# penumbra-zone/decaf377

Measured on AMD Instinct MI355X. Metric: decaf377 var-base scalar-mults/sec + encodes/sec at 1/2/4/8 MI355X, higher is better.
Workload: dtype u32

## Files before the change

decaf377_amd/csrc/curve.hpp:

```cpp
#pragma once
#include "fq29.hpp"
#include "fqs29.hpp"

namespace d377 {

#include "constants.inc"

constexpr int GT_STRIDE = 12;
constexpr int S_HASH_BITS = 12;
struct SqrtTables {
  const uint32_t* gtab;
  const uint8_t* s_lookup;
  uint32_t* inv_fail;
};

#include "s_hash.inc"

D377_HD uint32_t s_hash_raw(const fe& x) {
  return ((x.l[0] ^ (x.l[1] << 3)) * D377_S_HASH_K) >> (32 - S_HASH_BITS);
}
D377_HD uint32_t s_hash(const fe& x) {
  D377_B(bound_require(x.vq < 1.0535, "s_lookup key must be below q + 2^248"));
  return s_hash_raw(x);
}

D377_HD fe gt_load(const SqrtTables& T, int table, uint32_t idx) {
  const uint32_t* p = T.gtab + ((size_t)table * 256 + idx) * GT_STRIDE;
  fe r;
#if defined(__HIP_DEVICE_COMPILE__)
  const uint4* p4 = reinterpret_cast<const uint4*>(p);
  uint4 a = p4[0], b = p4[1], c = p4[2];
  r.l[0] = a.x; r.l[1] = a.y; r.l[2] = a.z; r.l[3] = a.w;
  r.l[4] = b.x; r.l[5] = b.y; r.l[6] = b.z; r.l[7] = b.w;
  r.l[8] = c.x;
#else
  for (int i = 0; i < NL; ++i) r.l[i] = p[i];
#endif
  fe_assume_carried(r, 1.1);
  return r;
}

D377_HD fe fe_sqr_n(fe x, int n) {
#pragma unroll 1
  for (int i = 0; i + 1 < n; i += 2) x = fe_sqr(fe_sqr(x));
  if (n & 1) x = fe_sqr(x);
  return x;
}

D377_HD fe fe_pow_2_47_m1(const fe& x) {
  fe e2 = fe_mul(fe_sqr(x), x);
  fe e4 = fe_mul(fe_sqr_n(e2, 2), e2);
  fe e5 = fe_mul(fe_sqr(e4), x);
  fe e10 = fe_mul(fe_sqr_n(e5, 5), e5);
  fe e11 = fe_mul(fe_sqr(e10), x);
  fe e22 = fe_mul(fe_sqr_n(e11, 11), e11);
  fe e23 = fe_mul(fe_sqr(e22), x);
  fe e46 = fe_mul(fe_sqr_n(e23, 23), e23);
  return fe_mul(fe_sqr(e46), x);
}

#ifndef D377_POW_W
#define D377_POW_W 4
#endif
#if D377_POW_W == 3
#define D377_POW_CHAIN POW_M12_CHAIN_W3
// ... 4 lines not shown
#define D377_POW_LEN D377_POW_M12_W4_LEN
#define D377_POW_TRAIL D377_POW_M12_W4_TRAILING_SQ
#endif
constexpr int POW_TAB = 1 << (D377_POW_W - 1);

struct RegPowTab {
  fe t[8];
  D377_HD void put(int j, const fe& v) { t[j] = v; }
  D377_HD fe get(int j) const {
    fe f;
    switch (j) {
      case 0: f = t[0]; break;
      case 1: f = t[1]; break;
      case 2: f = t[2]; break;
      case 3: f = t[3]; break;
      case 4: f = t[4]; break;
      case 5: f = t[5]; break;
      case 6: f = t[6]; break;
      default: f = t[7]; break;
    }
    return f;
  }
};

template <class PT>
D377_HD fe fe_pow_m12(const fe& x, PT& pt) {
  fe x2 = fe_sqr(x);
  fe cur = x;
  pt.put(0, cur);
#pragma unroll 1
  for (int j = 1; j < POW_TAB; ++j) {
    cur = fe_mul(cur, x2);
    pt.put(j, cur);
  }
  fe acc = pt.get((int)(D377_POW_CHAIN[0] & 15u) >> 1);
#pragma unroll 1
  for (int i = 1; i < D377_POW_LEN; ++i) {
    const uint32_t e = D377_POW_CHAIN[i];
    acc = fe_sqr_n(acc, (int)(e >> 4));
    acc = fe_mul(acc, pt.get((int)(e & 15u) >> 1));
  }
  return fe_sqr_n(acc, D377_POW_TRAIL);
}

D377_HD bool fe_strict_is_zero(const fe& a) {
  D377_B(bound_require(a.vq < 2.0, "fe_strict_is_zero needs a value below 2q"));
  uint32_t o = 0, d = 0;
#pragma unroll
  for (int i = 0; i < NL; ++i) { o |= a.l[i]; d |= a.l[i] ^ QL[i]; }
  return o == 0 || d == 0;
}

D377_HD bool fe_sqrt_tail(const SqrtTables& T, const fe& v, const fe& uv, bool den_zero, bool num_zero, fe* res, bool min_curve_root);

struct GivenPowers {
  fe v, uv;
  D377_HD void put(int, const fe&) {}
  D377_HD fe get(int) const { return fe_zero(); }
};
template <class PT> struct pt_has_powers { static constexpr bool value = false; };
template <> struct pt_has_powers<GivenPowers> { static constexpr bool value = true; };

template <bool NUM_IS_ONE, class PT>
D377_HD bool fe_sqrt_ratio_zeta(const SqrtTables& T, PT& pt, const fe& num, const fe& den, fe* res,
                                bool min_curve_root = false, const fe* inv_den = nullptr, bool use_inv = true) {
  const bool den_zero = fe_strict_is_zero(den);
  bool num_zero = false;
  if (!NUM_IS_ONE) num_zero = fe_strict_is_zero(num);

  fe v, uv;
  if constexpr (pt_has_powers<PT>::value) {
    v = pt.v;
    uv = pt.uv;
  } else if (inv_den != nullptr && use_inv) {
    const fe z = NUM_IS_ONE ? *inv_den : fe_mul(num, *inv_den);
    v = fe_pow_m12(z, pt);
    uv = fe_mul(v, z);
  } else {
    fe s = fe_pow_2_47_m1(den);
    fe t_ = fe_mul(fe_sqr(s), den);
    fe w = NUM_IS_ONE ? fe_mul(fe_pow_m12(t_, pt), s)
                      : fe_mul(fe_pow_m12(fe_mul(num, t_), pt), s);
    v = fe_mul(w, den);
    uv = NUM_IS_ONE ? w : fe_mul(w, num);
  }
  return fe_sqrt_tail(T, v, uv, den_zero, num_zero, res, min_curve_root);
}
D377_HD bool fe_sqrt_tail(const SqrtTables& T, const fe& v, const fe& uv, bool den_zero, bool num_zero, fe* res, bool min_curve_root) {
  fe x5 = fe_mul(uv, v);
  fe x4 = fe_sqr_n(x5, 8);
  fe x3 = fe_sqr_n(x4, 8);
  fe x2 = fe_sqr_n(x3, 8);
  fe x1 = fe_sqr_n(x2, 8);
  fe x0 = fe_sqr_strict(fe_sqr_strict(fe_sqr_n(x1, 5)));

  const uint64_t q0p = T.s_lookup[s_hash(x0)];
  uint64_t t = q0p;
  fe a1 = fe_mul_strict(x1, gt_load(T, 4, (uint32_t)(t & 0xFF)));
  t += (uint64_t)T.s_lookup[s_hash(a1)] << 7;
  fe a2 = fe_mul_strict(fe_mul(x2, gt_load(T, 3, (uint32_t)(t & 0xFF))),
                        gt_load(T, 4, (uint32_t)((t >> 8) & 0xFF)));
  t += (uint64_t)T.s_lookup[s_hash(a2)] << 15;
  fe a3 = fe_mul_strict(fe_mul(fe_mul(x3, gt_load(T, 2, (uint32_t)(t & 0xFF))),
                               gt_load(T, 3, (uint32_t)((t >> 8) & 0xFF))),
                        gt_load(T, 4, (uint32_t)((t >> 16) & 0xFF)));
  t += (uint64_t)T.s_lookup[s_hash(a3)] << 23;
  fe a4 = fe_mul_strict(fe_mul(fe_mul(fe_mul(x4, gt_load(T, 1, (uint32_t)(t & 0xFF))),
                                      gt_load(T, 2, (uint32_t)((t >> 8) & 0xFF))),
                               gt_load(T, 3, (uint32_t)((t >> 16) & 0xFF))),
                        gt_load(T, 4, (uint32_t)((t >> 24) & 0xFF)));
  t += (uint64_t)T.s_lookup[s_hash(a4)] << 31;
  fe a5 = fe_mul_strict(fe_mul(fe_mul(fe_mul(fe_mul(x5, gt_load(T, 0, (uint32_t)(t & 0xFF))),
                                             gt_load(T, 1, (uint32_t)((t >> 8) & 0xFF))),
                                      gt_load(T, 2, (uint32_t)((t >> 16) & 0xFF))),
                               gt_load(T, 3, (uint32_t)((t >> 24) & 0xFF))),
                        gt_load(T, 4, (uint32_t)((t >> 32) & 0xFF)));
  t += (uint64_t)T.s_lookup[s_hash(a5)] << 39;

  const uint64_t e2 = (D377_TS_U_INV * (t >> 1)) & ((1ull << 46) - 1);
  const bool flip = min_curve_root && (((D377_TS_U * e2) >> 46) & 1ull) != 0;
  t = (t + 1) >> 1;
  const bool nonsq = (q0p & 1) != 0;
  fe r = fe_select(nonsq, fe_mul(uv, fe_const(FE_NONSQUARE)), uv);
  r = fe_mul(r, gt_load(T, 0, (uint32_t)(t & 0xFF)));
  r = fe_mul(r, gt_load(T, 1, (uint32_t)((t >> 8) & 0xFF)));
  r = fe_mul(r, gt_load(T, 2, (uint32_t)((t >> 16) & 0xFF)));
  r = fe_mul(r, gt_load(T, 3, (uint32_t)((t >> 24) & 0xFF)));
  r = fe_mul(r, gt_load(T, 4, (uint32_t)((t >> 32) & 0xFF)));
  r = fe_mul(r, gt_load(T, 5, (uint32_t)((t >> 40) & 0xFF)));

  if (min_curve_root) r = fe_select(flip, fe_neg(r), r);
  bool was_square = !nonsq;
  if (den_zero) { r = fe_zero(); was_square = false; }
  if (num_zero) { r = fe_zero(); was_square = true; }
  *res = r;
  return was_square;
}

D377_HD fe fe_from_words_mod_order(const uint32_t w[8]) {
  return fe_mul(fe_from_words(w), fe_const(FE_R2));
}
D377_HD fe fe_from_words_mod_order_strict(const uint32_t w[8]) {
  return fe_mul_strict(fe_from_words(w), fe_const(FE_R2));
}
D377_HD fe fe_from_wide_words(const uint32_t lo[8], const uint32_t hi[8]) {
  return fe_add(fe_mul(fe_from_words(lo), fe_const(FE_R2)), fe_mul(fe_from_words(hi), fe_const(FE_R2_SHIFT256)));
}
D377_HD void fe_to_limbs28(const fe& x, uint32_t rec16[16]) {
  uint32_t w[8];
  fe_to_words(fe_canon(x), w);
#pragma unroll
  for (int k = 0; k < 10; ++k) {
    const int bit = 28 * k, lo = bit >> 5, sh = bit & 31;
// ... 275 lines not shown
}
template <class SQRT>
D377_HD uint32_t ge_decompress_with(const SqrtTables& T, const uint32_t w[8], ge* out, SQRT sqrt_of) {
  uint32_t bad = (w[7] >> 29) != 0;
  bad |= (uint32_t)words_geq(w, FQ_MODULUS_W_LIT);
  bad |= (w[0] & 1u);
  fe s = fe_mul(fe_from_words(w), fe_const(FE_R2));
  fe ss = fe_sqr(s);
  fe u1 = fe_sub(fe_const(FE_ONE), ss);
  fe u1sq = fe_sqr_strict(u1);
  fe u2 = fe_sub(u1sq, fe_mul(fe_const(FE_4D), ss));
  fe v;
  const bool was_square = sqrt_of(fe_mul_strict(u2, u1sq), &v);
  bad |= (uint32_t)!was_square;
  fe two_s_u1 = fe_mul(fe_dbl(s), u1);
  if (fe_is_negative(fe_mul(two_s_u1, v))) v = fe_neg(v);
  out->x = fe_mul(fe_mul(two_s_u1, fe_sqr(v)), u2);
  out->y = fe_mul(fe_mul(fe_add(fe_const(FE_ONE), ss), v), u1);
  out->z = fe_const(FE_ONE);
  out->t = fe_mul(out->x, out->y);
  D377_INVARIANT(T, *out, bad == 0);
  return bad;
}
template <class PT>
D377_HD uint32_t ge_decompress(const SqrtTables& T, PT& pt, const uint32_t w[8], ge* out, const fe* inv_den = nullptr) {
  return ge_decompress_with(T, w, out, [&](const fe& den, fe* v) {
    return fe_sqrt_ratio_zeta<true>(T, pt, fe_zero(), den, v, false, inv_den);
  });
}
D377_HD uint32_t ge_decompress_from_powers(const SqrtTables& T, const uint32_t w[8], const fe& pv, const fe& puv, ge* out) {
  return ge_decompress_with(T, w, out, [&](const fe& den, fe* v) {
    return fe_sqrt_tail(T, pv, puv, fe_strict_is_zero(den), false, v, false);
  });
}

D377_HD fe ge_compress_den(const ge& p) {
  fe u1 = fe_mul(fe_add(p.x, p.t), fe_sub(p.x, p.t));
  return fe_mul_strict(fe_mul(u1, fe_const(FE_A_MINUS_D)), fe_sqr(p.x));
}
template <class PT>
D377_HD void ge_compress(const SqrtTables& T, PT& pt, const ge& p, uint32_t w[8], bool is_element = true,
                         const fe* inv_den = nullptr) {
  D377_INVARIANT(T, p, is_element);
  const fe a_minus_d = fe_const(FE_A_MINUS_D);
  fe u1 = fe_mul(fe_add(p.x, p.t), fe_sub(p.x, p.t));
  fe v;
  (void)fe_sqrt_ratio_zeta<true>(T, pt, fe_zero(), fe_mul_strict(fe_mul(u1, a_minus_d), fe_sqr(p.x)), &v, false, inv_den);
  fe u2 = fe_abs(fe_mul(v, u1));
  fe u3 = fe_sub(fe_mul(u2, p.z), p.t);
  fe s = fe_mul(fe_mul(fe_mul(a_minus_d, v), u3), p.x);
// ... 218 lines not shown
  return r;
}

template <class F>
D377_HD ge_of<F> ge_double_neg(const ge_of<F>& p, bool with_t) {
  F a = fe_sqr(p.x), b = fe_sqr(p.y);
  F c = fe_sqr2x(p.z);
  F e = fe_mul(p.x, fe_dbl(p.y));
  F h = fe_add(a, b);
  F g = fe_sub(a, b);
  F f = fe_add(g, c);
  ge_of<F> r;
  r.x = fe_mul(e, f); r.y = fe_mul(g, h); r.z = fe_mul(f, g);
  r.t = p.t;
  if (with_t) r.t = fe_mul(e, h);
  return r;
}

D377_HD ge ge_double_latency(const ge& p) { return ge_double_fast(p, true); }

template <class F>
D377_HD gec_of<F> ge_to_cached(const ge_of<F>& p) {
  gec_of<F> c;
  c.ypx = fe_carry(fe_add(p.y, p.x));
  c.ymx = fe_sub(p.y, p.x);
  c.z2 = fe_dbl(p.z);
  c.kt = fe_mul(fe_as<F>(fe_const(FE_K)), p.t);
  return c;
}

template <class F>
D377_HD ge_of<F> ge_add_cached(const ge_of<F>& p, const gec_of<F>& q, bool neg, bool with_t) {
  F a = fe_mul(fe_sub_nc(p.y, p.x), q.ymx);
  F b = fe_mul(fe_add(p.y, p.x), q.ypx);
  F c = fe_mul(p.t, q.kt);
  F d = fe_mul(p.z, q.z2);
  F e = fe_sub(b, a), h = fe_add(b, a);
  F dmc = fe_sub(d, c), dpc = fe_add(d, c);
  F f = fe_select(neg, dpc, dmc), g = fe_select(neg, dmc, dpc);
  ge_of<F> r;
  r.x = fe_mul(e, f); r.y = fe_mul(g, h); r.z = fe_mul(f, g);
  r.t = p.t;
  if (with_t) r.t = fe_mul(e, h);
  return r;
}

struct gea { fe ypx, ymx, kt; };
// ... 10 lines not shown
  r.t = p.t;
  if (with_t) r.t = fe_mul(e, h);
  return r;
}

D377_HD gea gea_from_affine(const fe& x, const fe& y) {
  gea c;
  c.ypx = fe_carry(fe_add(y, x));
  c.ymx = fe_sub(y, x);
  c.kt = fe_mul(fe_mul(fe_const(FE_K), x), y);
  return c;
}
D377_HD ge ge_from_cached_affine(const gea& q, bool neg) {
  const fe one = fe_const(FE_ONE);
  ge r;
  r.x = fe_mul(fe_sub(q.ypx, fe_mul(q.ymx, one)), one);
  r.y = fe_mul(fe_add(q.ypx, q.ymx), one);
  r.z = fe_const(FE_TWO);
  const fe t = fe_mul(q.kt, fe_const(FE_2_OVER_K));
  r.t = fe_select(neg, fe_neg(t), t);
  return r;
}

template <class F = fe, class Tab>
D377_HD ge ge_scalar_mul_w4(const ge& p0, const uint32_t digits[8], Tab& tab, bool want_t = true) {
  const ge_of<F> p = ge_as<F>(p0);
  {
    gec_of<F> id;
    id.ypx = fe_as<F>(fe_const(FE_ONE)); id.ymx = fe_as<F>(fe_const(FE_ONE)); id.z2 = fe_dbl(fe_as<F>(fe_const(FE_ONE)));
    id.kt = fe_as<F>(fe_zero());
    tab.store(0, id);
  }
  const gec_of<F> pc = ge_to_cached(p);
  tab.store(1, pc);
  ge_of<F> acc = ge_double_fast(p, true);
  tab.store(2, ge_to_cached(acc));
#pragma unroll 1
  for (int j = 3; j <= 8; ++j) {
    acc = ge_add_cached(acc, pc, false, true);
    tab.store(j, ge_to_cached(acc));
  }
  int d = fr_digit(digits, 63);
  ge_of<F> r = ge_as<F>(ge_select(d != 0, p0, ge_identity()));
#pragma unroll 1
  for (int i = 62; i >= 0; --i) {
    d = fr_digit(digits, i);
    const bool neg = d < 0;
    const gec_of<F> e = tab.load(neg ? -d : d, neg);
#pragma unroll 1
    for (int j = 0; j < 4; ++j) r = ge_double_neg(r, j == 3);
    r = ge_add_cached(r, e, neg, want_t && i == 0);
  }
  return ge_unsigned(r);
}

// ... 302 lines not shown
```

decaf377_amd/csrc/d377.hip:

```cpp
#include <hip/hip_runtime.h>
#include <stdint.h>
#include <stdio.h>
#include <stdlib.h>
#include <string.h>
#include <chrono>
#include <mutex>
#include <new>
#include <string>
#include <thread>
#include <type_traits>
#include <vector>

#include "../../include/decaf377_amd.h"
#include "curve.hpp"
#include "device_util.hpp"
#include "dcb.hpp"
#include "quad_ops.hpp"
#include "row_ops.hpp"
#include "host_state.hpp"
#include "codec_chunked.hpp"
#include "fixed_comb.hpp"

using namespace d377;

thread_local char d377_g_err[512] = "";

namespace {

template <class F>
struct GlobalTab {
  uint32_t* base;
  size_t nthreads, tid;
  __device__ __forceinline__ void store(int j, const gec_of<F>& c) {
    uint32_t* p = base + ((size_t)j * nthreads + tid) * VB_ENTRY_WORDS;
    slot_store(p, c.ypx); slot_store(p + SLOT, c.ymx); slot_store(p + 2 * SLOT, c.z2); slot_store(p + 3 * SLOT, c.kt);
  }
  __device__ __forceinline__ gec_of<F> load(int j, bool swap) const {
    const uint32_t* p = base + ((size_t)j * nthreads + tid) * VB_ENTRY_WORDS;
    gec_of<F> c;
    c.ypx = slot_load_as<F>(p + (swap ? SLOT : 0));
    c.ymx = slot_load_as<F>(p + (swap ? 0 : SLOT));
    c.z2 = slot_load_as<F>(p + 2 * SLOT);
    c.kt = slot_load_as<F>(p + 3 * SLOT);
    return c;
  }
};
template <int BITS>
struct FixedTab {
  const uint32_t* base;
  __device__ __forceinline__ gea load(int i, int j, bool swap) const {
    return pt_load_affine(base + ((size_t)i * FbShape<BITS>::entries + j) * FBW_ENTRY_WORDS, swap);
  }
};

__device__ fe fe_pow_u32(const fe& x, uint32_t e) {
  int top = 31 - __clz((int)e);
  fe r = x;
#pragma unroll 1
  for (int i = top - 1; i >= 0; --i) {
    r = fe_sqr(r);
    if ((e >> i) & 1u) r = fe_mul(r, x);
  }
  return r;
}

__global__ void __launch_bounds__(BLOCK) k_init_gtab(uint32_t* gtab) {
  const int idx = blockIdx.x * BLOCK + threadIdx.x;
  if (idx >= 6 * 256) return;
  const int t = idx >> 8, nu = idx & 255;
  fe base = fe_sqr_n(fe_const(FE_SQRT_G), 8 * t);
  fe v = nu == 0 ? fe_const(FE_ONE) : fe_pow_u32(base, (uint32_t)nu);
  v = fe_mul_strict(v, fe_const(FE_ONE));
  uint32_t* p = gtab + (size_t)idx * GT_STRIDE;
#pragma unroll
  for (int i = 0; i < NL; ++i) p[i] = v.l[i];
  p[9] = 0; p[10] = 0; p[11] = 0;
}

__global__ void __launch_bounds__(BLOCK) k_init_slookup(uint8_t* s_lookup, uint32_t* keys ,
                                                        int* collisions) {
  const int nu = threadIdx.x;
  fe b39 = fe_sqr_n(fe_const(FE_SQRT_G_INV), 39);
  fe v = nu == 0 ? fe_const(FE_ONE) : fe_pow_u32(b39, (uint32_t)nu);
  fe c = fe_reduce_once(fe_mul_strict(v, fe_const(FE_ONE)));
  keys[2 * nu] = s_hash_raw(c);
  uint32_t h2 = 0xFFFFFFFFu;
  if (c.l[NL - 1] < (1u << 16)) {
    fe cq = fe_add(c, fe_const(Q_LIMBS));
    uint32_t carry = 0;
    fe n;
#pragma unroll
    for (int i = 0; i < NL; ++i) {
      uint32_t t = cq.l[i] + carry;
      if (i < NL - 1) { n.l[i] = t & MASK29; carry = t >> RB; } else n.l[i] = t;
    }
    h2 = s_hash_raw(n);
  }
  keys[2 * nu + 1] = h2;
  for (int i = threadIdx.x; i < (1 << S_HASH_BITS); i += BLOCK) s_lookup[i] = 0;
// ... 204 lines not shown
        io.put(3, j, w);
      }
    },
    [&](DcbIO& io2, int cnt) {
      if (__any(flagged != 0)) {
#pragma unroll 1
        for (int j = 0; j < cnt; ++j) {
          const bool mine = ((flagged >> j) & 1u) != 0;
          if (!__any(mine)) continue;
          Words8 a1, a2;
          io2.get(2, j, a1.w);
          io2.get(3, j, a2.w);
          const Words8 r = hash_exceptional_words(T, pt, a1, a2);
          if (mine) io2.emit(j, r.w);
        }
      }
      flagged = 0;
    });
  D377_DCB_END();
}

__global__ void __launch_bounds__(BLOCK, WAVES_PER_SIMD) k_scalar_mul_var(SqrtTables T, const uint8_t* enc32,
                                                          const uint8_t* scalar32, size_t n, uint8_t* out32,
                                                          uint8_t* status, uint32_t* scratch, DcbScratch dcb) {
  D377_POW_LDS();
  D377_DCB_BEGIN(out32);
  GlobalTab<fes> tab;
  tab.base = scratch;
  tab.nthreads = (size_t)dcb.nslots * BLOCK;
  tab.tid = io.lane;
  dcb_rounds<1, true, false>(n, io, pt,
    [&](size_t i, int j) {
      uint32_t w[8];
      load32(enc32, i, w);
      dcb_put_den(io, 0, j, ge_decompress_den(w));
    },
    [&](size_t i, int j, const uint32_t (*invw)[8], bool have) {
      uint32_t w[8], k[8], dg[8];
      load32(enc32, i, w);
      load32(scalar32, i, k);
      const fe inv = fe_from_words(invw[0]);
      ge g;
      const uint32_t bad = ge_decompress(T, pt, w, &g, &inv);
      status[i] = (uint8_t)bad;
      fr_reduce_words(k);
      fr_half_words(k);
      fr_recode_signed16(k, dg);
      const ge r = ge_scalar_mul_w4<fes>(g, dg, tab, DCB_WANT_T);
      D377_INVARIANT(T, r, bad == 0);
      dcb_put(io, j, ge_dcb_from_half(r, bad != 0));
    });
  D377_DCB_END();
}

template <int BITS>
__global__ void __launch_bounds__(BLOCK, FB_SETS) k_scalar_mul_base(SqrtTables T, const uint32_t* fbase,
                                                           const uint8_t* scalar32, size_t n, uint8_t* out32, DcbScratch dcb) {
  D377_POW_LDS();
  D377_DCB_BEGIN(out32);
  FixedTab<BITS> ft{fbase};
  dcb_rounds<0, true>(n, io, pt,
    [&](size_t, int) {},
    [&](size_t i, int j, const uint32_t (*)[8], bool) {
      uint32_t k[8];
      load32(scalar32, i, k);
      fr_reduce_words(k);
// ... 381 lines not shown
  const size_t e_raw = (size_t)blockIdx.x * 2 + ((t >> 1) & 1);
  const size_t e = e_raw < n ? e_raw : n - 1;
  uint32_t w[8];
  load32(which ? r2 : r1, e, w);
  const fe r0 = fe_from_words_mod_order(w);
  fe s_own, t_own;
  GivenPowers pt = tiny4_powers<false>(L, fe_zero(), ge_elligator_den(r0), K);
  ge_elligator_st(T, pt, r0, &s_own, &t_own);
  D377_INVARIANT(T, ge_from_jacobi_st(s_own, t_own), t < 4);
  const fe s_oth = fe_quad_perm<1, 0, 3, 2>(s_own), t_oth = fe_quad_perm<1, 0, 3, 2>(t_own);
  const bool second = which != 0;
  bool exceptional;
  dcb_state st = ge_dcb_from_jacobi_sum(fe_select(second, s_oth, s_own), fe_select(second, t_oth, t_own),
                                        fe_select(second, s_own, s_oth), fe_select(second, t_own, t_oth), &exceptional);
#if defined(D377_CHECK_INVARIANTS)
  exceptional |= (e & 3) == 3;
#endif
  if (__any(exceptional)) tiny_hash_exceptional(T, r1, r2, e, exceptional, st);
  tiny4_encode(st, w);
  if (t < 4 && which == 0 && e_raw < n) store32(out32, e, w);
}

__global__ void __launch_bounds__(BLOCK, WAVES_PER_SIMD) k_scalar_mul_var_el(const uint64_t* xyzt, const uint8_t* scalar32, size_t n,
                                                                             uint64_t* out, uint32_t* scratch, DcbScratch dcb) {
  const int slot = dcb_claim(dcb);
  if (slot < 0) return;
  GlobalTab<fes> tab;
  tab.base = scratch;
  tab.nthreads = (size_t)dcb.nslots * BLOCK;
  tab.tid = (size_t)slot * BLOCK + threadIdx.x;
  const size_t chunk_elems = (size_t)dcb.per_lane * BLOCK;
  for (size_t chunk = blockIdx.x; chunk * chunk_elems < n; chunk += gridDim.x) {
    if (chunk != blockIdx.x && threadIdx.x == 0)
      atomicExch(dcb.pool + slot, (int)(atomicAdd(dcb.health, 1u) & 0x7FFFFFFFu) + 1);
#pragma unroll 1
    for (int j = 0; j < dcb.per_lane; ++j) {
      const size_t i = chunk * chunk_elems + (size_t)j * BLOCK + threadIdx.x;
      if (i >= n) break;
      dcb_progress_priority(dcb.prio, j, dcb.per_lane);
      uint32_t k[8], dg[8];
      load32(scalar32, i, k);
      const ge g = load_ge_mont256(xyzt, i);
      fr_reduce_words(k);
      fr_recode_signed16(k, dg);
      store_ge_mont256(out, i, ge_scalar_mul_w4<fes>(g, dg, tab));
    }
  }
  dcb_release(dcb, slot);
}
template <int BITS>
__global__ void __launch_bounds__(BLOCK, WAVES_PER_SIMD) k_scalar_mul_base_el(const uint32_t* fbase, const uint8_t* scalar32, size_t n,
// ... 468 lines not shown
    return fail(D377_ERR_NO_DEVICE, "device is %s, this library is built for gfx950 only", prop.gcnArchName);
  d.cus = prop.multiProcessorCount;
  HIP_TRY(hipStreamCreateWithFlags(&d.stream, hipStreamNonBlocking));
  HIP_TRY(hipStreamCreateWithFlags(&d.copy_stream, hipStreamNonBlocking));
  {
    int least = 0, greatest = 0;
    HIP_TRY(hipDeviceGetStreamPriorityRange(&least, &greatest));
    HIP_TRY(hipStreamCreateWithPriority(&d.ctl_stream, hipStreamNonBlocking, greatest));
  }
  for (int i = 0; i < 2; ++i) {
    HIP_TRY(hipEventCreateWithFlags(&d.ev_in[i], hipEventDisableTiming));
    HIP_TRY(hipEventCreateWithFlags(&d.ev_done[i], hipEventDisableTiming));
  }
  HIP_TRY(hipEventCreateWithFlags(&d.ev_shard, hipEventDisableTiming));
  int rc;
  if ((rc = d.vb_guard.init()) || (rc = d.msm.guard.init())) return rc;
  HIP_TRY(hipMalloc(&d.gtab, (size_t)6 * 256 * GT_STRIDE * sizeof(uint32_t)));
  HIP_TRY(hipMalloc(&d.s_lookup, (size_t)1 << S_HASH_BITS));
  HIP_TRY(hipMalloc(&d.inv_fail, sizeof(uint32_t)));
  HIP_TRY(hipMemsetAsync(d.inv_fail, 0, sizeof(uint32_t), d.stream));
  d.vb_blocks = d.cus * WAVES_PER_SIMD;

  HIP_TRY(hipMalloc(&d.vb_scratch, (size_t)d.vb_blocks * BLOCK * VB_ENTRIES * VB_ENTRY_WORDS * sizeof(uint32_t)));
  for (int k = 0; k < CK_COUNT; ++k) { d.chunk_sets[k] = WAVES_PER_SIMD; d.chunk_k[k] = DCB_K; }
  d.chunk_sets[CK_MUL_BASE] = FB_SETS;
  d.chunk_k[CK_MUL_BASE] = FB_K;
  d.dcb_sets = d.cus * DCB_SETS_MAX;
  HIP_TRY(hipMalloc(&d.dcb_scratch, (size_t)d.dcb_sets * BLOCK * DCB_SLOTS * DCB_KMAX * 32));
  HIP_TRY(hipMalloc(&d.slot_pool, (size_t)d.dcb_sets * sizeof(int)));
  HIP_TRY(hipMemsetAsync(d.slot_pool, 0, (size_t)d.dcb_sets * sizeof(int), d.stream));
  HIP_TRY(hipMalloc(&d.pool_health, 4 * sizeof(uint32_t)));
  HIP_TRY(hipMemsetAsync(d.pool_health, 0, 4 * sizeof(uint32_t), d.stream));
  HIP_TRY(hipHostMalloc(&d.starve_host, 2 * sizeof(uint32_t), hipHostMallocDefault));
  d.starve_host[0] = d.starve_host[1] = 0;
  HIP_TRY(hipHostMalloc(&d.pool_host, ((size_t)d.dcb_sets + 4) * sizeof(int), hipHostMallocDefault));
  if ((rc = check_residency(d))) return rc;
  uint32_t* keys = nullptr;
  int* coll = nullptr;
  HIP_TRY(hipMalloc(&keys, 512 * sizeof(uint32_t)));
  if (hipMalloc(&coll, sizeof(int)) != hipSuccess) { (void)hipFree(keys); return fail(D377_ERR_HIP, "%s", "hipMalloc failed"); }
  rc = init_tables(d, keys, coll);
  (void)hipFree(keys);
  (void)hipFree(coll);
  if (rc == D377_OK && !d.fb_lazy) rc = ensure_comb(d, nullptr);
  return rc;
}

void free_device(DeviceState& d) {
  if (d.id < 0) return;
  (void)hipSetDevice(d.id);
  if (d.stream) (void)hipStreamSynchronize(d.stream);
  if (d.copy_stream) (void)hipStreamSynchronize(d.copy_stream);
  (void)d.vb_guard.drain();
  (void)d.msm.guard.drain();
  (void)hipFree(d.gtab); (void)hipFree(d.s_lookup); (void)hipFree(d.fbase); (void)hipFree(d.fb_bases); (void)hipFree(d.bm_scratch); (void)hipFree(d.vb_scratch); (void)hipFree(d.dcb_scratch); (void)hipFree(d.slot_pool); (void)hipFree(d.pool_health); (void)hipFree(d.inv_fail);
  if (d.starve_host) (void)hipHostFree(d.starve_host);
  d.starve_host = nullptr;
  if (d.pool_host) (void)hipHostFree(d.pool_host);
  d.pool_host = nullptr;
  for (int i = 0; i < 4; ++i) { (void)hipFree(d.buf[i]); (void)hipFree(d.buf2[i]); (void)hipFree(d.shard[i]); }
  for (int i = 0; i < 2; ++i) {
    if (d.ev_in[i]) (void)hipEventDestroy(d.ev_in[i]);
    if (d.ev_done[i]) (void)hipEventDestroy(d.ev_done[i]);
  }
  if (d.ev_shard) (void)hipEventDestroy(d.ev_shard);
  d.vb_guard.destroy();
  d.msm.guard.destroy();
  if (d.copy_stream) (void)hipStreamDestroy(d.copy_stream);
  if (d.ctl_stream) (void)hipStreamDestroy(d.ctl_stream);
  (void)hipFree(d.msm.mem);
  for (uint8_t* r : d.msm.retired) (void)hipFree(r);
  d.msm.retired.clear();
  if (d.stream) (void)hipStreamDestroy(d.stream);
}

int launch(DeviceState& d, hipStream_t s, Op op, int aux, const void* in0, const void* in1, size_t n, void* out0, void* out1) {
  if (n == 0) return D377_OK;
  const SqrtTables T = d.tables();
// ... 101 lines not shown
      DcbScratch db;
      chunks_of(wide ? FB_SETS : WAVES_PER_SIMD, fk, gb, db);
      if (wide && gb > d.cus * FB_SETS) db.prio = 0;
      if ((rc = vb.acquire())) return rc;
      if ((rc = with_fb_bits(d.fb_bits, [&](auto b) -> int {
             hipLaunchKernelGGL((k_scalar_mul_base<decltype(b)::value>), dim3(gb), dim3(BLOCK), wide ? d.chunk_lds[CK_MUL_BASE] : d.fb_narrow_lds, s, T, d.fbase,
                                (const uint8_t*)in0, n, (uint8_t*)out0, db);
             return D377_OK; }))) return rc;
      break;
    }
    case OP_MUL_VAR:
      if (n <= tiny_batch_max(d)) {
        hipLaunchKernelGGL(k_scalar_mul_var_tiny<false>, dim3((unsigned)n), dim3(64), 0, s, T, (const uint8_t*)in0, (const uint8_t*)in1, n,
                           (uint8_t*)out0, (uint8_t*)out1);
        break;
      }
      if (n <= small_batch_max(d, false)) {
        hipLaunchKernelGGL(k_scalar_mul_var_small<false>, dim3((unsigned)((n + SMALL_QUADS - 1) / SMALL_QUADS)), dim3(SMALL_THREADS), 0, s, T,
                           (const uint8_t*)in0, (const uint8_t*)in1, n, (uint8_t*)out0, (uint8_t*)out1);
        break;
      }
      if ((rc = vb.acquire())) return rc;
      hipLaunchKernelGGL(k_scalar_mul_var, dim3(gv), dim3(BLOCK), d.chunk_lds[CK_MUL_VAR], s, T, (const uint8_t*)in0, (const uint8_t*)in1, n,
                         (uint8_t*)out0, (uint8_t*)out1, d.vb_scratch, dcb);
      break;
    case OP_ENCODE:
      if (n <= tiny4_batch_max(d)) {
        hipLaunchKernelGGL(k_map_to_curve_tiny, dim3(tiny4_grid(n)), dim3(64), 0, s, T, (const uint8_t*)in0, (const uint8_t*)nullptr, n, (uint8_t*)out0);
        break;
      }
      if ((rc = vb.acquire())) return rc;
      hipLaunchKernelGGL(k_encode_to_curve, dim3(gv), dim3(BLOCK), d.chunk_lds[CK_ENCODE], s, T, (const uint8_t*)in0, n, (uint8_t*)out0, dcb);
      break;
    case OP_HASH:
      if (n <= tiny4_batch_max(d) / 2) {
        hipLaunchKernelGGL(k_hash_to_curve_tiny2, dim3((unsigned)((n + 1) / 2)), dim3(64), 0, s, T, (const uint8_t*)in0, (const uint8_t*)in1, n, (uint8_t*)out0);
        break;
      }
      if (n <= tiny4_batch_max(d)) {
        hipLaunchKernelGGL(k_map_to_curve_tiny, dim3(tiny4_grid(n)), dim3(64), 0, s, T, (const uint8_t*)in0, (const uint8_t*)in1, n, (uint8_t*)out0);
        break;
      }
      if ((rc = vb.acquire())) return rc;
      hipLaunchKernelGGL(k_hash_to_curve, dim3(gv), dim3(BLOCK), d.chunk_lds[CK_HASH], s, T, (const uint8_t*)in0, (const uint8_t*)in1, n,
                         (uint8_t*)out0, dcb);
      break;
    case OP_ADD:
// ... 46 lines not shown
      break;
    case OP_NEG:
      hipLaunchKernelGGL(k_neg, dim3(g), dim3(BLOCK), 0, s, (const uint64_t*)in0, n, (uint64_t*)out0);
      break;
    case OP_MUL_VAR_EL: {
      if (n <= tiny_batch_max(d)) {
        hipLaunchKernelGGL(k_scalar_mul_var_tiny<true>, dim3((unsigned)n), dim3(64), 0, s, T, (const uint8_t*)in0, (const uint8_t*)in1, n,
                           (uint8_t*)out0, (uint8_t*)nullptr);
        break;
      }
      if (n <= small_batch_max(d, true)) {
        hipLaunchKernelGGL(k_scalar_mul_var_small<true>, dim3((unsigned)((n + SMALL_QUADS - 1) / SMALL_QUADS)), dim3(SMALL_THREADS), 0, s, T,
                           (const uint8_t*)in0, (const uint8_t*)in1, n, (uint8_t*)out0, (uint8_t*)nullptr);
        break;
      }
      DcbScratch dv = dcb;
      dv.extra = 0;
      dv.per_lane = n > d.resident_lanes() ? 2 : 1;
      size_t nch = (n + (size_t)dv.per_lane * BLOCK - 1) / ((size_t)dv.per_lane * BLOCK);
      if (nch > (size_t)d.cus * 64) nch = (size_t)d.cus * 64;
      dv.prio = nch <= 2 * (size_t)d.cus * WAVES_PER_SIMD ? 1 : 0;
      if ((rc = vb.acquire())) return rc;
      hipLaunchKernelGGL(k_scalar_mul_var_el, dim3((int)nch), dim3(BLOCK), d.chunk_lds[CK_MUL_VAR_EL], s, (const uint64_t*)in0, (const uint8_t*)in1, n,
                         (uint64_t*)out0, d.vb_scratch, dv);
      break;
    }
    case OP_MUL_BASE_EL:
      if ((rc = ensure_comb(d, s))) return rc;
      if ((rc = with_fb_bits(d.fb_bits, [&](auto b) -> int {
             constexpr int BITS = decltype(b)::value;
             if (n <= tiny_batch_max(d))
               hipLaunchKernelGGL((k_scalar_mul_base_tiny<true, BITS>), dim3((unsigned)n), dim3(64), 0, s, d.fbase, (const uint8_t*)in0, n, (uint8_t*)out0);
             else if (n <= small_batch_max(d, true))
               hipLaunchKernelGGL((k_scalar_mul_base_small<true, BITS>), dim3((unsigned)((n + SMALL_QUADS - 1) / SMALL_QUADS)), dim3(SMALL_THREADS), 0, s, d.fbase,
                                  (const uint8_t*)in0, n, (uint8_t*)out0);
             else
               hipLaunchKernelGGL((k_scalar_mul_base_el<BITS>), dim3(g), dim3(BLOCK), 0, s, d.fbase, (const uint8_t*)in0, n, (uint64_t*)out0);
             return D377_OK; }))) return rc;
      break;
    case OP_COMPRESS_FIELD:
      hipLaunchKernelGGL(k_compress_to_field, dim3(g), dim3(BLOCK), 0, s, T, (const uint64_t*)in0, n, (uint64_t*)out0);
      break;
    case OP_ENCODE_EL:
    case OP_HASH_EL:
      if ((rc = vb.acquire())) return rc;
      hipLaunchKernelGGL(k_map_to_element, dim3(gv), dim3(BLOCK), d.chunk_lds[CK_MAP_EL], s, T, (const uint8_t*)in0,
                         op == OP_HASH_EL ? (const uint8_t*)in1 : (const uint8_t*)nullptr, n, (uint64_t*)out0, dcb);
// ... 805 lines not shown
```

decaf377_amd/csrc/device_util.hpp:

```cpp
#pragma once
#include <hip/hip_runtime.h>
#include <stdint.h>

#include "curve.hpp"

namespace d377 {

constexpr int BLOCK = 256;
#ifndef D377_WAVES_PER_SIMD
#define D377_WAVES_PER_SIMD 2
#endif
constexpr int WAVES_PER_SIMD = D377_WAVES_PER_SIMD;
constexpr int SLOT = 12;
constexpr int VB_ENTRIES = 9;
constexpr int VB_ENTRY_WORDS = 4 * SLOT;
constexpr int AP_WORDS = 32;
constexpr int FBW_ENTRY_WORDS = AP_WORDS;

__device__ __forceinline__ void load32(const uint8_t* base, size_t i, uint32_t w[8]) {
  const uint4* p = reinterpret_cast<const uint4*>(base) + 2 * i;
  uint4 a = p[0], b = p[1];
  w[0] = a.x; w[1] = a.y; w[2] = a.z; w[3] = a.w; w[4] = b.x; w[5] = b.y; w[6] = b.z; w[7] = b.w;
}
__device__ __forceinline__ void store32(uint8_t* base, size_t i, const uint32_t w[8]) {
// ... 94 lines not shown
    c.ymx.l[i] = swap ? w[i] : w[NL + i];
    c.kt.l[i] = w[2 * NL + i];
  }
  return c;
}
__device__ __forceinline__ gea pt_load_affine(const uint32_t* p, bool swap) { return gea_from_raw(pt_load_affine_raw(p), swap); }
__device__ __forceinline__ void gea_pin(gea& c) {
#pragma unroll
  for (int i = 0; i < NL; ++i) asm volatile("" : "+v"(c.ypx.l[i]), "+v"(c.ymx.l[i]), "+v"(c.kt.l[i]) : : "memory");
}

struct LdsPowTab {
  uint32_t* col;
  __device__ __forceinline__ void put(int j, const fe& v) {
#pragma unroll
    for (int k = 0; k < NL; ++k) col[(j * NL + k) * BLOCK] = v.l[k];
  }
  __device__ __forceinline__ fe get(int j) const {
    fe r;
#pragma unroll
    for (int k = 0; k < NL; ++k) r.l[k] = col[(j * NL + k) * BLOCK];
    return r;
  }
};
constexpr int REC_TILE_CHUNKS = 64 * 8;
__device__ __forceinline__ int rec_swz(int c) { return (c & ~7) | ((c & 7) ^ ((c >> 3) & 7)); }
__device__ __forceinline__ void rec_lds_fence() { asm volatile("s_waitcnt lgkmcnt(0)" ::: "memory"); }
__device__ __forceinline__ void wave_load_records128(const uint64_t* base, size_t rec0, size_t n, uint4* tile, int lane, uint32_t w[32]) {
  const uint4* g = reinterpret_cast<const uint4*>(base) + 8 * rec0;
  const size_t left = n - rec0;
  const int chunks = left >= 64 ? REC_TILE_CHUNKS : (int)left * 8;
  uint4 r[8];
#pragma unroll
  for (int k = 0; k < 8; ++k) { const int c = k * 64 + lane; r[k] = c < chunks ? g[c] : make_uint4(0, 0, 0, 0); }
#pragma unroll
  for (int k = 0; k < 8; ++k) tile[rec_swz(k * 64 + lane)] = r[k];
  rec_lds_fence();
#pragma unroll
  for (int k = 0; k < 8; ++k) { const uint4 v = tile[rec_swz(lane * 8 + k)]; w[4 * k] = v.x; w[4 * k + 1] = v.y; w[4 * k + 2] = v.z; w[4 * k + 3] = v.w; }
  rec_lds_fence();
}
__device__ __forceinline__ void wave_store_records128(uint64_t* base, size_t rec0, size_t n, uint4* tile, int lane, const uint32_t w[32]) {
  uint4* g = reinterpret_cast<uint4*>(base) + 8 * rec0;
  const size_t left = n - rec0;
  const int chunks = left >= 64 ? REC_TILE_CHUNKS : (int)left * 8;
#pragma unroll
// ... 20 lines not shown
```

decaf377_amd/csrc/host_state.hpp:

```cpp
#pragma once
#include <hip/hip_runtime.h>
#include <stdint.h>
#include <stdio.h>
#include <string.h>
#include <mutex>
#include <vector>

#include "../../include/decaf377_amd.h"
#include "curve.hpp"
#include "device_util.hpp"

extern thread_local char d377_g_err[512];

namespace d377 {

inline int fail(int code, const char* fmt, const char* detail) {
  snprintf(d377_g_err, sizeof d377_g_err, fmt, detail);
  return code;
}
#define HIP_TRY(expr)                                                                     \
  do {                                                                                    \
    hipError_t e_ = (expr);                                                               \
    if (e_ != hipSuccess) return ::d377::fail(D377_ERR_HIP, #expr ": %s", hipGetErrorString(e_)); \
  } while (0)
// ... 44 lines not shown
  int id = -1;
  int cus = 0;
  int chunk_lds[CK_COUNT] = {0, 0, 0, 0, 0, 0, 0, 0};
  int chunk_blocks[CK_COUNT] = {0, 0, 0, 0, 0, 0, 0, 0};
  int chunk_sets[CK_COUNT] = {0, 0, 0, 0, 0, 0, 0, 0};
  int chunk_k[CK_COUNT] = {0, 0, 0, 0, 0, 0, 0, 0};
  int fb_narrow_lds = 0;
  int msm_enc_chunked = -1;
  int codec_chunked = -1;
  int msm_span_blocks = -1;
  int dcb_sets = 0;
  uint32_t* bm_scratch = nullptr;
  size_t bm_cap = 0;
  int bm_lds[2] = {-1, -1};
  int fx_lds[4] = {-1, -1, -1, -1};
  int fxi_lds[4] = {-1, -1, -1, -1};
  uint32_t* gtab = nullptr;
  uint8_t* s_lookup = nullptr;
  uint32_t* fbase = nullptr;
  uint32_t* fb_bases = nullptr;
  int fb_bits = FB_BITS;
  bool fb_lazy = false;
  uint32_t* vb_scratch = nullptr;
  uint8_t* dcb_scratch = nullptr;
  int* slot_pool = nullptr;
  uint32_t* pool_health = nullptr;
  int* pool_host = nullptr;
  uint32_t* starve_host = nullptr;
  int vb_blocks = 0;
  uint32_t* inv_fail = nullptr;
  ScratchGuard vb_guard;
  hipStream_t stream = nullptr;
  hipStream_t copy_stream = nullptr;
  hipStream_t ctl_stream = nullptr;
  hipEvent_t ev_in[2] = {nullptr, nullptr}, ev_done[2] = {nullptr, nullptr};
  uint8_t* buf[4] = {nullptr, nullptr, nullptr, nullptr};
  size_t cap[4] = {0, 0, 0, 0};
  uint8_t* buf2[4] = {nullptr, nullptr, nullptr, nullptr};
  size_t cap2[4] = {0, 0, 0, 0};
  uint8_t* shard[4] = {nullptr, nullptr, nullptr, nullptr};
  size_t shard_cap[4] = {0, 0, 0, 0};
  hipEvent_t ev_shard = nullptr;
  MsmWorkspace msm;
  const Tuning* tune = nullptr;
  long long tuned(int key, long long dflt) const { return (tune && tune->v[key] >= 0) ? tune->v[key] : dflt; }
  bool is_tuned(int key) const { return tune && tune->v[key] >= 0; }
// ... 92 lines not shown
```

Baseline: 72.22 million.

## Run var-base sqrt pow chain in signed limbs and share identity table entry

The sqrt-ratio power chain, the tail's table multiplies and the final root product are templated on the field type. The var-base scalar-mult path now runs them in the signed-limb representation (fes), converting to unsigned only where strict or hashed values are needed. This is meant to cut carry/reduction work in the long squaring chain. The per-thread identity entry of the global window table is replaced by one shared device record, which removes a per-lane scratch store. The to-cached conversion also skips a carry for signed limbs. These changes lean on bound assumptions for the signed representation and add a table-load select on j.

```diff
diff --git a/decaf377_amd/csrc/curve.hpp b/decaf377_amd/csrc/curve.hpp
--- a/decaf377_amd/csrc/curve.hpp
+++ b/decaf377_amd/csrc/curve.hpp
@@ -24,7 +24,8 @@
   return s_hash_raw(x);
 }
 
-D377_HD fe gt_load(const SqrtTables& T, int table, uint32_t idx) {
+template <class F = fe>
+D377_HD F gt_load(const SqrtTables& T, int table, uint32_t idx) {
   const uint32_t* p = T.gtab + ((size_t)table * 256 + idx) * GT_STRIDE;
   fe r;
 #if defined(__HIP_DEVICE_COMPILE__)
@@ -37,10 +38,11 @@
   for (int i = 0; i < NL; ++i) r.l[i] = p[i];
 #endif
   fe_assume_carried(r, 1.1);
-  return r;
-}
-
-D377_HD fe fe_sqr_n(fe x, int n) {
+  return fe_as<F>(r);
+}
+
+template <class F>
+D377_HD F fe_sqr_n(F x, int n) {
 #pragma unroll 1
   for (int i = 0; i + 1 < n; i += 2) x = fe_sqr(fe_sqr(x));
   if (n & 1) x = fe_sqr(x);
@@ -91,23 +93,33 @@
     return f;
   }
 };
-
-template <class PT>
-D377_HD fe fe_pow_m12(const fe& x, PT& pt) {
-  fe x2 = fe_sqr(x);
-  fe cur = x;
+struct RegPowTabS {
+  fes t[8];
+  D377_HD void put(int j, const fes& v) { t[j] = v; }
+  D377_HD fes get_signed(int j) const { return t[j & 7]; }
+};
+template <class F, class PT>
+D377_HD F pt_get(const PT& pt, int j) {
+  if constexpr (std::is_same<F, fe>::value) return pt.get(j);
+  else return pt.get_signed(j);
+}
+
+template <class F = fe, class PT>
+D377_HD F fe_pow_m12(const F& x, PT& pt) {
+  F x2 = fe_sqr(x);
+  F cur = x;
   pt.put(0, cur);
 #pragma unroll 1
   for (int j = 1; j < POW_TAB; ++j) {
     cur = fe_mul(cur, x2);
     pt.put(j, cur);
   }
-  fe acc = pt.get((int)(D377_POW_CHAIN[0] & 15u) >> 1);
+  F acc = pt_get<F>(pt, (int)(D377_POW_CHAIN[0] & 15u) >> 1);
 #pragma unroll 1
   for (int i = 1; i < D377_POW_LEN; ++i) {
     const uint32_t e = D377_POW_CHAIN[i];
     acc = fe_sqr_n(acc, (int)(e >> 4));
-    acc = fe_mul(acc, pt.get((int)(e & 15u) >> 1));
+    acc = fe_mul(acc, pt_get<F>(pt, (int)(e & 15u) >> 1));
   }
   return fe_sqr_n(acc, D377_POW_TRAIL);
 }
@@ -120,7 +132,8 @@
   return o == 0 || d == 0;
 }
 
-D377_HD bool fe_sqrt_tail(const SqrtTables& T, const fe& v, const fe& uv, bool den_zero, bool num_zero, fe* res, bool min_curve_root);
+template <class F>
+D377_HD bool fe_sqrt_tail(const SqrtTables& T, const F& v, const F& uv, bool den_zero, bool num_zero, fe* res, bool min_curve_root);
 
 struct GivenPowers {
   fe v, uv;
@@ -130,59 +143,60 @@
 template <class PT> struct pt_has_powers { static constexpr bool value = false; };
 template <> struct pt_has_powers<GivenPowers> { static constexpr bool value = true; };
 
-template <bool NUM_IS_ONE, class PT>
+template <bool NUM_IS_ONE, class F = fe, class PT>
 D377_HD bool fe_sqrt_ratio_zeta(const SqrtTables& T, PT& pt, const fe& num, const fe& den, fe* res,
                                 bool min_curve_root = false, const fe* inv_den = nullptr, bool use_inv = true) {
   const bool den_zero = fe_strict_is_zero(den);
   bool num_zero = false;
   if (!NUM_IS_ONE) num_zero = fe_strict_is_zero(num);
 
-  fe v, uv;
+  F v, uv;
   if constexpr (pt_has_powers<PT>::value) {
-    v = pt.v;
-    uv = pt.uv;
+    v = fe_as<F>(pt.v);
+    uv = fe_as<F>(pt.uv);
   } else if (inv_den != nullptr && use_inv) {
-    const fe z = NUM_IS_ONE ? *inv_den : fe_mul(num, *inv_den);
-    v = fe_pow_m12(z, pt);
+    const F z = fe_as<F>(NUM_IS_ONE ? *inv_den : fe_mul(num, *inv_den));
+    v = fe_pow_m12<F>(z, pt);
     uv = fe_mul(v, z);
   } else {
     fe s = fe_pow_2_47_m1(den);
     fe t_ = fe_mul(fe_sqr(s), den);
-    fe w = NUM_IS_ONE ? fe_mul(fe_pow_m12(t_, pt), s)
-                      : fe_mul(fe_pow_m12(fe_mul(num, t_), pt), s);
-    v = fe_mul(w, den);
-    uv = NUM_IS_ONE ? w : fe_mul(w, num);
+    F w = NUM_IS_ONE ? fe_mul(fe_pow_m12<F>(fe_as<F>(t_), pt), fe_as<F>(s))
+                     : fe_mul(fe_pow_m12<F>(fe_as<F>(fe_mul(num, t_)), pt), fe_as<F>(s));
+    v = fe_mul(w, fe_as<F>(den));
+    uv = NUM_IS_ONE ? w : fe_mul(w, fe_as<F>(num));
   }
   return fe_sqrt_tail(T, v, uv, den_zero, num_zero, res, min_curve_root);
 }
-D377_HD bool fe_sqrt_tail(const SqrtTables& T, const fe& v, const fe& uv, bool den_zero, bool num_zero, fe* res, bool min_curve_root) {
-  fe x5 = fe_mul(uv, v);
-  fe x4 = fe_sqr_n(x5, 8);
-  fe x3 = fe_sqr_n(x4, 8);
-  fe x2 = fe_sqr_n(x3, 8);
-  fe x1 = fe_sqr_n(x2, 8);
-  fe x0 = fe_sqr_strict(fe_sqr_strict(fe_sqr_n(x1, 5)));
+template <class F>
+D377_HD bool fe_sqrt_tail(const SqrtTables& T, const F& v, const F& uv, bool den_zero, bool num_zero, fe* res, bool min_curve_root) {
+  F x5 = fe_mul(uv, v);
+  F x4 = fe_sqr_n(x5, 8);
+  F x3 = fe_sqr_n(x4, 8);
+  F x2 = fe_sqr_n(x3, 8);
+  F x1 = fe_sqr_n(x2, 8);
+  fe x0 = fe_sqr_strict(fe_sqr_strict(fe_unsigned(fe_sqr_n(x1, 5))));
 
   const uint64_t q0p = T.s_lookup[s_hash(x0)];
   uint64_t t = q0p;
-  fe a1 = fe_mul_strict(x1, gt_load(T, 4, (uint32_t)(t & 0xFF)));
+  fe a1 = fe_mul_strict(fe_unsigned(x1), gt_load(T, 4, (uint32_t)(t & 0xFF)));
   t += (uint64_t)T.s_lookup[s_hash(a1)] << 7;
-  fe a2 = fe_mul_strict(fe_mul(x2, gt_load(T, 3, (uint32_t)(t & 0xFF))),
+  fe a2 = fe_mul_strict(fe_unsigned(fe_mul(x2, gt_load<F>(T, 3, (uint32_t)(t & 0xFF)))),
                         gt_load(T, 4, (uint32_t)((t >> 8) & 0xFF)));
   t += (uint64_t)T.s_lookup[s_hash(a2)] << 15;
-  fe a3 = fe_mul_strict(fe_mul(fe_mul(x3, gt_load(T, 2, (uint32_t)(t & 0xFF))),
-                               gt_load(T, 3, (uint32_t)((t >> 8) & 0xFF))),
+  fe a3 = fe_mul_strict(fe_unsigned(fe_mul(fe_mul(x3, gt_load<F>(T, 2, (uint32_t)(t & 0xFF))),
+                                           gt_load<F>(T, 3, (uint32_t)((t >> 8) & 0xFF)))),
                         gt_load(T, 4, (uint32_t)((t >> 16) & 0xFF)));
   t += (uint64_t)T.s_lookup[s_hash(a3)] << 23;
-  fe a4 = fe_mul_strict(fe_mul(fe_mul(fe_mul(x4, gt_load(T, 1, (uint32_t)(t & 0xFF))),
-                                      gt_load(T, 2, (uint32_t)((t >> 8) & 0xFF))),
-                               gt_load(T, 3, (uint32_t)((t >> 16) & 0xFF))),
+  fe a4 = fe_mul_strict(fe_unsigned(fe_mul(fe_mul(fe_mul(x4, gt_load<F>(T, 1, (uint32_t)(t & 0xFF))),
+                                                  gt_load<F>(T, 2, (uint32_t)((t >> 8) & 0xFF))),
+                                           gt_load<F>(T, 3, (uint32_t)((t >> 16) & 0xFF)))),
                         gt_load(T, 4, (uint32_t)((t >> 24) & 0xFF)));
   t += (uint64_t)T.s_lookup[s_hash(a4)] << 31;
-  fe a5 = fe_mul_strict(fe_mul(fe_mul(fe_mul(fe_mul(x5, gt_load(T, 0, (uint32_t)(t & 0xFF))),
-                                             gt_load(T, 1, (uint32_t)((t >> 8) & 0xFF))),
-                                      gt_load(T, 2, (uint32_t)((t >> 16) & 0xFF))),
-                               gt_load(T, 3, (uint32_t)((t >> 24) & 0xFF))),
+  fe a5 = fe_mul_strict(fe_unsigned(fe_mul(fe_mul(fe_mul(fe_mul(x5, gt_load<F>(T, 0, (uint32_t)(t & 0xFF))),
+                                                         gt_load<F>(T, 1, (uint32_t)((t >> 8) & 0xFF))),
+                                                  gt_load<F>(T, 2, (uint32_t)((t >> 16) & 0xFF))),
+                                           gt_load<F>(T, 3, (uint32_t)((t >> 24) & 0xFF)))),
                         gt_load(T, 4, (uint32_t)((t >> 32) & 0xFF)));
   t += (uint64_t)T.s_lookup[s_hash(a5)] << 39;
 
@@ -190,14 +204,15 @@
   const bool flip = min_curve_root && (((D377_TS_U * e2) >> 46) & 1ull) != 0;
   t = (t + 1) >> 1;
   const bool nonsq = (q0p & 1) != 0;
-  fe r = fe_select(nonsq, fe_mul(uv, fe_const(FE_NONSQUARE)), uv);
-  r = fe_mul(r, gt_load(T, 0, (uint32_t)(t & 0xFF)));
-  r = fe_mul(r, gt_load(T, 1, (uint32_t)((t >> 8) & 0xFF)));
-  r = fe_mul(r, gt_load(T, 2, (uint32_t)((t >> 16) & 0xFF)));
-  r = fe_mul(r, gt_load(T, 3, (uint32_t)((t >> 24) & 0xFF)));
-  r = fe_mul(r, gt_load(T, 4, (uint32_t)((t >> 32) & 0xFF)));
-  r = fe_mul(r, gt_load(T, 5, (uint32_t)((t >> 40) & 0xFF)));
-
+  F rf = fe_select(nonsq, fe_mul(uv, fe_as<F>(fe_const(FE_NONSQUARE))), uv);
+  rf = fe_mul(rf, gt_load<F>(T, 0, (uint32_t)(t & 0xFF)));
+  rf = fe_mul(rf, gt_load<F>(T, 1, (uint32_t)((t >> 8) & 0xFF)));
+  rf = fe_mul(rf, gt_load<F>(T, 2, (uint32_t)((t >> 16) & 0xFF)));
+  rf = fe_mul(rf, gt_load<F>(T, 3, (uint32_t)((t >> 24) & 0xFF)));
+  rf = fe_mul(rf, gt_load<F>(T, 4, (uint32_t)((t >> 32) & 0xFF)));
+  rf = fe_mul(rf, gt_load<F>(T, 5, (uint32_t)((t >> 40) & 0xFF)));
+
+  fe r = fe_unsigned(rf);
   if (min_curve_root) r = fe_select(flip, fe_neg(r), r);
   bool was_square = !nonsq;
   if (den_zero) { r = fe_zero(); was_square = false; }
@@ -519,10 +534,10 @@
   D377_INVARIANT(T, *out, bad == 0);
   return bad;
 }
-template <class PT>
+template <class F = fe, class PT>
 D377_HD uint32_t ge_decompress(const SqrtTables& T, PT& pt, const uint32_t w[8], ge* out, const fe* inv_den = nullptr) {
   return ge_decompress_with(T, w, out, [&](const fe& den, fe* v) {
-    return fe_sqrt_ratio_zeta<true>(T, pt, fe_zero(), den, v, false, inv_den);
+    return fe_sqrt_ratio_zeta<true, F>(T, pt, fe_zero(), den, v, false, inv_den);
   });
 }
 D377_HD uint32_t ge_decompress_from_powers(const SqrtTables& T, const uint32_t w[8], const fe& pv, const fe& puv, ge* out) {
@@ -787,7 +802,8 @@
 template <class F>
 D377_HD gec_of<F> ge_to_cached(const ge_of<F>& p) {
   gec_of<F> c;
-  c.ypx = fe_carry(fe_add(p.y, p.x));
+  if constexpr (std::is_same<F, fes>::value) c.ypx = fe_add(p.y, p.x);
+  else c.ypx = fe_carry(fe_add(p.y, p.x));
   c.ymx = fe_sub(p.y, p.x);
   c.z2 = fe_dbl(p.z);
   c.kt = fe_mul(fe_as<F>(fe_const(FE_K)), p.t);
@@ -844,15 +860,20 @@
   return r;
 }
 
+template <class F>
+D377_HD gec_of<F> gec_identity() {
+  gec_of<F> id;
+  id.ypx = fe_as<F>(fe_const(FE_ONE)); id.ymx = fe_as<F>(fe_const(FE_ONE)); id.z2 = fe_dbl(fe_as<F>(fe_const(FE_ONE)));
+  id.kt = fe_as<F>(fe_zero());
+  return id;
+}
+template <class Tab, class = void> struct tab_shares_identity { static constexpr bool value = false; };
+template <class Tab> struct tab_shares_identity<Tab, std::void_t<decltype(Tab::shared_identity)>> { static constexpr bool value = Tab::shared_identity; };
+
 template <class F = fe, class Tab>
 D377_HD ge ge_scalar_mul_w4(const ge& p0, const uint32_t digits[8], Tab& tab, bool want_t = true) {
   const ge_of<F> p = ge_as<F>(p0);
-  {
-    gec_of<F> id;
-    id.ypx = fe_as<F>(fe_const(FE_ONE)); id.ymx = fe_as<F>(fe_const(FE_ONE)); id.z2 = fe_dbl(fe_as<F>(fe_const(FE_ONE)));
-    id.kt = fe_as<F>(fe_zero());
-    tab.store(0, id);
-  }
+  if constexpr (!tab_shares_identity<Tab>::value) tab.store(0, gec_identity<F>());
   const gec_of<F> pc = ge_to_cached(p);
   tab.store(1, pc);
   ge_of<F> acc = ge_double_fast(p, true);
diff --git a/decaf377_amd/csrc/d377.hip b/decaf377_amd/csrc/d377.hip
--- a/decaf377_amd/csrc/d377.hip
+++ b/decaf377_amd/csrc/d377.hip
@@ -29,14 +29,17 @@
 
 template <class F>
 struct GlobalTab {
+  static constexpr bool shared_identity = true;
   uint32_t* base;
+  const uint32_t* ident;
   size_t nthreads, tid;
   __device__ __forceinline__ void store(int j, const gec_of<F>& c) {
     uint32_t* p = base + ((size_t)j * nthreads + tid) * VB_ENTRY_WORDS;
     slot_store(p, c.ypx); slot_store(p + SLOT, c.ymx); slot_store(p + 2 * SLOT, c.z2); slot_store(p + 3 * SLOT, c.kt);
   }
   __device__ __forceinline__ gec_of<F> load(int j, bool swap) const {
-    const uint32_t* p = base + ((size_t)j * nthreads + tid) * VB_ENTRY_WORDS;
+    const uint32_t* own = base + ((size_t)j * nthreads + tid) * VB_ENTRY_WORDS;
+    const uint32_t* p = j == 0 ? ident : own;
     gec_of<F> c;
     c.ypx = slot_load_as<F>(p + (swap ? SLOT : 0));
     c.ymx = slot_load_as<F>(p + (swap ? 0 : SLOT));
@@ -75,6 +78,12 @@
 #pragma unroll
   for (int i = 0; i < NL; ++i) p[i] = v.l[i];
   p[9] = 0; p[10] = 0; p[11] = 0;
+}
+
+__global__ void k_init_vb_identity(uint32_t* rec) {
+  if (blockIdx.x != 0 || threadIdx.x != 0) return;
+  const gec_of<fes> id = gec_identity<fes>();
+  slot_store(rec, id.ypx); slot_store(rec + SLOT, id.ymx); slot_store(rec + 2 * SLOT, id.z2); slot_store(rec + 3 * SLOT, id.kt);
 }
 
 __global__ void __launch_bounds__(BLOCK) k_init_slookup(uint8_t* s_lookup, uint32_t* keys ,
@@ -325,11 +334,13 @@
 
 __global__ void __launch_bounds__(BLOCK, WAVES_PER_SIMD) k_scalar_mul_var(SqrtTables T, const uint8_t* enc32,
                                                           const uint8_t* scalar32, size_t n, uint8_t* out32,
-                                                          uint8_t* status, uint32_t* scratch, DcbScratch dcb) {
+                                                          uint8_t* status, uint32_t* scratch, const uint32_t* vb_identity,
+                                                          DcbScratch dcb) {
   D377_POW_LDS();
   D377_DCB_BEGIN(out32);
   GlobalTab<fes> tab;
   tab.base = scratch;
+  tab.ident = vb_identity;
   tab.nthreads = (size_t)dcb.nslots * BLOCK;
   tab.tid = io.lane;
   dcb_rounds<1, true, false>(n, io, pt,
@@ -344,7 +355,7 @@
       load32(scalar32, i, k);
       const fe inv = fe_from_words(invw[0]);
       ge g;
-      const uint32_t bad = ge_decompress(T, pt, w, &g, &inv);
+      const uint32_t bad = ge_decompress<fes>(T, pt, w, &g, &inv);
       status[i] = (uint8_t)bad;
       fr_reduce_words(k);
       fr_half_words(k);
@@ -772,11 +783,13 @@
 }
 
 __global__ void __launch_bounds__(BLOCK, WAVES_PER_SIMD) k_scalar_mul_var_el(const uint64_t* xyzt, const uint8_t* scalar32, size_t n,
-                                                                             uint64_t* out, uint32_t* scratch, DcbScratch dcb) {
+                                                                             uint64_t* out, uint32_t* scratch, const uint32_t* vb_identity,
+                                                                             DcbScratch dcb) {
   const int slot = dcb_claim(dcb);
   if (slot < 0) return;
   GlobalTab<fes> tab;
   tab.base = scratch;
+  tab.ident = vb_identity;
   tab.nthreads = (size_t)dcb.nslots * BLOCK;
   tab.tid = (size_t)slot * BLOCK + threadIdx.x;
   const size_t chunk_elems = (size_t)dcb.per_lane * BLOCK;
@@ -1291,6 +1304,9 @@
   d.vb_blocks = d.cus * WAVES_PER_SIMD;
 
   HIP_TRY(hipMalloc(&d.vb_scratch, (size_t)d.vb_blocks * BLOCK * VB_ENTRIES * VB_ENTRY_WORDS * sizeof(uint32_t)));
+  HIP_TRY(hipMalloc(&d.vb_identity, VB_ENTRY_WORDS * sizeof(uint32_t)));
+  hipLaunchKernelGGL(k_init_vb_identity, dim3(1), dim3(64), 0, d.stream, d.vb_identity);
+  HIP_TRY(hipGetLastError());
   for (int k = 0; k < CK_COUNT; ++k) { d.chunk_sets[k] = WAVES_PER_SIMD; d.chunk_k[k] = DCB_K; }
   d.chunk_sets[CK_MUL_BASE] = FB_SETS;
   d.chunk_k[CK_MUL_BASE] = FB_K;
@@ -1322,7 +1338,7 @@
   if (d.copy_stream) (void)hipStreamSynchronize(d.copy_stream);
   (void)d.vb_guard.drain();
   (void)d.msm.guard.drain();
-  (void)hipFree(d.gtab); (void)hipFree(d.s_lookup); (void)hipFree(d.fbase); (void)hipFree(d.fb_bases); (void)hipFree(d.bm_scratch); (void)hipFree(d.vb_scratch); (void)hipFree(d.dcb_scratch); (void)hipFree(d.slot_pool); (void)hipFree(d.pool_health); (void)hipFree(d.inv_fail);
+  (void)hipFree(d.gtab); (void)hipFree(d.s_lookup); (void)hipFree(d.fbase); (void)hipFree(d.fb_bases); (void)hipFree(d.bm_scratch); (void)hipFree(d.vb_scratch); (void)hipFree(d.vb_identity); (void)hipFree(d.dcb_scratch); (void)hipFree(d.slot_pool); (void)hipFree(d.pool_health); (void)hipFree(d.inv_fail);
   if (d.starve_host) (void)hipHostFree(d.starve_host);
   d.starve_host = nullptr;
   if (d.pool_host) (void)hipHostFree(d.pool_host);
@@ -1470,7 +1486,7 @@
       }
       if ((rc = vb.acquire())) return rc;
       hipLaunchKernelGGL(k_scalar_mul_var, dim3(gv), dim3(BLOCK), d.chunk_lds[CK_MUL_VAR], s, T, (const uint8_t*)in0, (const uint8_t*)in1, n,
-                         (uint8_t*)out0, (uint8_t*)out1, d.vb_scratch, dcb);
+                         (uint8_t*)out0, (uint8_t*)out1, d.vb_scratch, (const uint32_t*)d.vb_identity, dcb);
       break;
     case OP_ENCODE:
       if (n <= tiny4_batch_max(d)) {
@@ -1563,7 +1579,7 @@
       dv.prio = nch <= 2 * (size_t)d.cus * WAVES_PER_SIMD ? 1 : 0;
       if ((rc = vb.acquire())) return rc;
       hipLaunchKernelGGL(k_scalar_mul_var_el, dim3((int)nch), dim3(BLOCK), d.chunk_lds[CK_MUL_VAR_EL], s, (const uint64_t*)in0, (const uint8_t*)in1, n,
-                         (uint64_t*)out0, d.vb_scratch, dv);
+                         (uint64_t*)out0, d.vb_scratch, (const uint32_t*)d.vb_identity, dv);
       break;
     }
     case OP_MUL_BASE_EL:
diff --git a/decaf377_amd/csrc/device_util.hpp b/decaf377_amd/csrc/device_util.hpp
--- a/decaf377_amd/csrc/device_util.hpp
+++ b/decaf377_amd/csrc/device_util.hpp
@@ -140,6 +140,16 @@
     for (int k = 0; k < NL; ++k) r.l[k] = col[(j * NL + k) * BLOCK];
     return r;
   }
+  __device__ __forceinline__ void put(int j, const fes& v) {
+#pragma unroll
+    for (int k = 0; k < NL; ++k) col[(j * NL + k) * BLOCK] = (uint32_t)v.l[k];
+  }
+  __device__ __forceinline__ fes get_signed(int j) const {
+    fes r;
+#pragma unroll
+    for (int k = 0; k < NL; ++k) r.l[k] = (int32_t)col[(j * NL + k) * BLOCK];
+    return r;
+  }
 };
 constexpr int REC_TILE_CHUNKS = 64 * 8;
 __device__ __forceinline__ int rec_swz(int c) { return (c & ~7) | ((c & 7) ^ ((c >> 3) & 7)); }
diff --git a/decaf377_amd/csrc/host_state.hpp b/decaf377_amd/csrc/host_state.hpp
--- a/decaf377_amd/csrc/host_state.hpp
+++ b/decaf377_amd/csrc/host_state.hpp
@@ -90,6 +90,7 @@
   int fb_bits = FB_BITS;
   bool fb_lazy = false;
   uint32_t* vb_scratch = nullptr;
+  uint32_t* vb_identity = nullptr;
   uint8_t* dcb_scratch = nullptr;
   int* slot_pool = nullptr;
   uint32_t* pool_health = nullptr;
```

Result: faster. 73.07 million, median of 6 (+1.2%).
